# victorramirez952/tomography_3d_reconstructor

Hardware: AMD Instinct MI355X
Metric: Mvoxels/s (SDF+MC) on 1024^3 ellipsoid stack; achieved HBM GB/s vs peak (higher is better)
Workload: dtype f64

## Files before the change

### include/tomo_hip.h

```cpp
#ifndef TOMO_HIP_H
#define TOMO_HIP_H

#include <stddef.h>
#include <stdint.h>

#ifdef __cplusplus
extern "C" {
#endif

#define TOMO_OK 0
#define TOMO_E_ARG (-1)
#define TOMO_E_LAUNCH (-2)
#define TOMO_E_SIZE (-3)
#define TOMO_E_WORKSPACE (-4)

int tomo_abi_version(void);
const char *tomo_error_string(int code);
int tomo_host_mc_cell(const float *h_v, double iso, int8_t *h_tris, int *h_uses_centre);
double tomo_host_mc_edge_offset(double va, double vb);
void tomo_host_mc_centre_offset(const double *h_v8, double *h_out3);

int tomo_host_checksum(const void *h_data, int64_t nbytes, int nthreads, uint64_t *h_out);
int tomo_host_checksum_impl(const void *h_data, int64_t nbytes, int nthreads, int impl, uint64_t *h_out);
int64_t tomo_host_checksum_chunk_bytes(void);
// ... 64 lines not shown
int64_t tomo_mc_scan_workspace_bytes(int64_t n);
int tomo_mc_scan(const uint32_t *counts, int64_t n, uint32_t *off_a, uint32_t *off_b, uint32_t *nz_ids,
                 unsigned long long *totals, void *workspace, int64_t workspace_bytes, void *stream);
int tomo_mc_list(int Nz, int Ny, int Nx, int xorg, const uint32_t *seg_aoff, const unsigned long long *seg_act,
                 unsigned long long *vox_key, void *stream);
int tomo_mc_eval(const float *field, int Nz, int Ny, int Nx, int64_t pitch, int xorg, double iso,
                 const unsigned long long *vox_key, int64_t na, uint32_t *vox_counts, uint8_t *vox_flags, void *stream);
int tomo_mc_list_capped(int Nz, int Ny, int Nx, int xorg, const uint32_t *seg_aoff, const unsigned long long *seg_act,
                        unsigned long long *vox_key, int64_t cap, void *stream);
int tomo_mc_eval_capped(const float *field, int Nz, int Ny, int Nx, int64_t pitch, int xorg, double iso,
                        const unsigned long long *vox_key, int64_t cap, const unsigned long long *na_dev,
                        uint32_t *vox_counts, uint8_t *vox_flags, void *stream);
int tomo_mc_emit(const float *field, int Nz, int Ny, int Nx, int64_t pitch, int xorg, double iso,
                 const unsigned long long *vox_key, int64_t na, const unsigned long long *seg_act,
                 const uint32_t *seg_aoff, const uint32_t *vox_voff, const uint32_t *vox_foff, const uint8_t *vox_flags,
                 int z_offset, unsigned long long *vkey, float *vpos, int32_t *faces, unsigned long long *totals,
                 void *stream);

int tomo_mc_first_touch(const float *field, int Nz, int Ny, int Nx, int64_t pitch, int xorg, double iso,
                        const unsigned long long *vox_key, int64_t na, const unsigned long long *seg_act,
                        const uint32_t *seg_aoff, const uint32_t *vox_voff, const uint8_t *vox_flags, int mode,
                        uint32_t *created, const uint32_t *base, int32_t *ft_rank, unsigned long long *totals, void *stream);

int tomo_mc3_list(int Nz, int Ny, int Nx, int xorg, const uint32_t *seg_cnt, const unsigned long long *seg_act,
                  uint32_t *seg_blk, uint32_t *seg_aoff, unsigned long long *vox_key, int64_t cap, unsigned long long *tot,
                  void *stream);
int tomo_mc3_eval(const float *field, int Nz, int Ny, int Nx, int64_t pitch, int xorg, double iso,
                  const unsigned long long *vox_key, int64_t cap, const unsigned long long *tot, int z_offset,
                  uint32_t *vox_loc, int32_t *vox_til, uint8_t *vox_flags, uint16_t *vox_used, float *vox_f3, float *vox_c3,
                  uint32_t *blk3, void *stream);
int64_t tomo_mc3_slice_table_words(int Nz, int Ny);
int64_t tomo_mc3_sort_segments(int Nz, int Ny);
int tomo_mc3_scan(int Nz, int Ny, int Nx, int xorg, const uint32_t *seg_aoff, const uint32_t *vox_loc, int64_t cap,
                  uint32_t *blk3, uint32_t *slice_tab, unsigned long long *tot, int64_t cap_v, int64_t cap_f, void *stream);
int tomo_mc3_vertices(int Nz, int Ny, int Nx, int xorg, const unsigned long long *vox_key, int64_t cap,
                      const unsigned long long *tot, const uint32_t *vox_loc, const uint8_t *vox_flags, const float *vox_f3,
                      const float *vox_c3, const uint32_t *blk3, const uint32_t *slice_tab, int z_offset, int shift,
                      const double *cum, int64_t ncum, const double *adj, int64_t nadj, float mm_y, float mm_x, float *vrec,
                      uint32_t *keys, uint32_t *idx, void *stream);
int64_t tomo_mc3_sort_workspace_bytes(int64_t cap_v, int64_t nseg);
int tomo_mc3_sort_rank_top(const float *vrec, uint32_t *keys, uint32_t *idx, int64_t cap_v, int Nz, int Ny, const uint32_t *slice_tab,
                           unsigned long long *tot, float *uniq, int32_t *table, void *workspace, int64_t workspace_bytes,
                           float z_top, void *stream);
int tomo_mc3_sort_rank_fused(const float *vrec, const uint32_t *keys, int64_t cap_v, int Nz, int Ny, uint32_t *slice_tab,
                             unsigned long long *tot, float *uniq, int32_t *table, float z_top, void *stream);
int tomo_mc3_faces(int Nz, int Ny, int Nx, int xorg, const unsigned long long *vox_key, int64_t cap, unsigned long long *tot,
// ... 55 lines not shown
```

### tomography_3d_reconstructor_amd/_lib.py

```python
import ctypes
import os
import subprocess

_HERE = os.path.dirname(os.path.abspath(__file__))
SO_PATH = os.environ.get("TOMO_LIB") or os.path.join(_HERE, "libtomo_hip.so")
CSRC = os.path.join(_HERE, "csrc")

_c_i = ctypes.c_int
_c_i64 = ctypes.c_int64
_c_p = ctypes.c_void_p
_c_d = ctypes.c_double
_c_f = ctypes.c_float

SIGNATURES = {
    "tomo_abi_version": (_c_i, []),
    "tomo_error_string": (ctypes.c_char_p, [_c_i]),
    "tomo_host_mc_cell": (_c_i, [_c_p, _c_d, _c_p, _c_p]),
    "tomo_host_mc_edge_offset": (_c_d, [_c_d, _c_d]),
    "tomo_host_mc_centre_offset": (None, [_c_p, _c_p]),
    "tomo_host_checksum": (_c_i, [_c_p, _c_i64, _c_i, _c_p]),
    "tomo_host_checksum_impl": (_c_i, [_c_p, _c_i64, _c_i, _c_i, _c_p]),
    "tomo_host_checksum_chunk_bytes": (_c_i64, []),
    "tomo_host_checksum_part": (_c_i, [_c_p, _c_i64, _c_i64, _c_i, _c_i, _c_p]),
    "tomo_host_checksum_fold": (_c_i, [_c_p, _c_i64, _c_i64, _c_p]),
# ... 33 lines not shown
    "tomo_morph_fused": (_c_i, [_c_p, _c_p, _c_i, _c_i, _c_i, ctypes.c_uint32, _c_i, _c_p]),
    "tomo_smooth": (_c_i, [_c_p, _c_p, _c_i, _c_i, _c_i, _c_i, _c_i, _c_p]),
    "tomo_extend_bits": (_c_i, [_c_p, _c_p, _c_i, _c_i, _c_i, _c_i, _c_p]),
    "tomo_field_fill": (_c_i, [_c_p, _c_p, _c_i, _c_i, _c_i, _c_i, _c_i, _c_p, _c_p, _c_p]),
    "tomo_field_fill_bits": (_c_i, [_c_p, _c_p, _c_i, _c_i, _c_i, _c_i, _c_p, _c_p, _c_p]),
    "tomo_field_span_bytes": (_c_i64, [_c_i, _c_i, _c_i, _c_i]),
    "tomo_field_fill_bits_sparse": (_c_i, [_c_p, _c_p, _c_i, _c_i, _c_i, _c_i, _c_p, _c_p, _c_p, _c_p]),
    "tomo_sign_rows": (_c_i64, [_c_i]),
    "tomo_field_signs_fused": (_c_i, [_c_i]),
    "tomo_sign_buffer_words": (_c_i64, [_c_i, _c_i, _c_i, _c_i]),
    "tomo_field_signs": (_c_i, [_c_p, _c_i, _c_i, _c_i, _c_i64, _c_i, _c_d, _c_i, _c_i, _c_p, _c_p, _c_p]),
    "tomo_mc_classify": (_c_i, [_c_p, _c_p, _c_i, _c_i, _c_i, _c_i, _c_p, _c_p, _c_p]),
    "tomo_mc_scan_segments": (_c_i, [_c_p, _c_i64, _c_p, _c_p, _c_p, _c_i64, _c_p]),
    "tomo_mc_scan_workspace_bytes": (_c_i64, [_c_i64]),
    "tomo_mc_scan": (_c_i, [_c_p, _c_i64, _c_p, _c_p, _c_p, _c_p, _c_p, _c_i64, _c_p]),
    "tomo_mc_list": (_c_i, [_c_i, _c_i, _c_i, _c_i, _c_p, _c_p, _c_p, _c_p]),
    "tomo_mc_eval": (_c_i, [_c_p, _c_i, _c_i, _c_i, _c_i64, _c_i, _c_d, _c_p, _c_i64, _c_p, _c_p, _c_p]),
    "tomo_mc_list_capped": (_c_i, [_c_i, _c_i, _c_i, _c_i, _c_p, _c_p, _c_p, _c_i64, _c_p]),
    "tomo_mc_eval_capped": (_c_i, [_c_p, _c_i, _c_i, _c_i, _c_i64, _c_i, _c_d, _c_p, _c_i64, _c_p, _c_p, _c_p, _c_p]),
    "tomo_mc_emit": (_c_i, [_c_p, _c_i, _c_i, _c_i, _c_i64, _c_i, _c_d, _c_p, _c_i64, _c_p, _c_p, _c_p, _c_p, _c_p, _c_i, _c_p,
                            _c_p, _c_p, _c_p, _c_p]),
    "tomo_mc_first_touch": (_c_i, [_c_p, _c_i, _c_i, _c_i, _c_i64, _c_i, _c_d, _c_p, _c_i64, _c_p, _c_p, _c_p, _c_p, _c_i, _c_p,
                                   _c_p, _c_p, _c_p, _c_p]),
    "tomo_mc3_list": (_c_i, [_c_i, _c_i, _c_i, _c_i, _c_p, _c_p, _c_p, _c_p, _c_p, _c_i64, _c_p, _c_p]),
    "tomo_mc3_eval": (_c_i, [_c_p, _c_i, _c_i, _c_i, _c_i64, _c_i, _c_d, _c_p, _c_i64, _c_p, _c_i, _c_p, _c_p, _c_p, _c_p, _c_p,
                             _c_p, _c_p, _c_p]),
    "tomo_mc3_slice_table_words": (_c_i64, [_c_i, _c_i]),
    "tomo_mc3_sort_segments": (_c_i64, [_c_i, _c_i]),
    "tomo_mc3_scan": (_c_i, [_c_i, _c_i, _c_i, _c_i, _c_p, _c_p, _c_i64, _c_p, _c_p, _c_p, _c_i64, _c_i64, _c_p]),
    "tomo_mc3_vertices": (_c_i, [_c_i, _c_i, _c_i, _c_i, _c_p, _c_i64, _c_p, _c_p, _c_p, _c_p, _c_p, _c_p, _c_p, _c_i, _c_i,
                                 _c_p, _c_i64, _c_p, _c_i64, _c_f, _c_f, _c_p, _c_p, _c_p, _c_p]),
    "tomo_mc3_sort_workspace_bytes": (_c_i64, [_c_i64, _c_i64]),
    "tomo_mc3_sort_rank_top": (_c_i, [_c_p, _c_p, _c_p, _c_i64, _c_i, _c_i, _c_p, _c_p, _c_p, _c_p, _c_p, _c_i64, _c_f, _c_p]),
    "tomo_mc3_sort_rank_fused": (_c_i, [_c_p, _c_p, _c_i64, _c_i, _c_i, _c_p, _c_p, _c_p, _c_p, _c_f, _c_p]),
    "tomo_mc3_faces": (_c_i, [_c_i, _c_i, _c_i, _c_i, _c_p, _c_i64, _c_p, _c_p, _c_p, _c_p, _c_p, _c_p, _c_p, _c_p, _c_p, _c_i64, _c_p]),
    "tomo_vertex_finalize": (_c_i, [_c_p, _c_i64, _c_i, _c_p, _c_i64, _c_p, _c_i64, _c_f, _c_f, _c_p]),
    "tomo_mesh_unique_workspace_bytes": (_c_i64, [_c_i64]),
    "tomo_mesh_unique": (_c_i, [_c_p, _c_i64, _c_p, _c_p, _c_p, _c_p, _c_i64, _c_p]),
    "tomo_mesh_lookup": (_c_i, [_c_p, _c_i64, _c_p, _c_i64, _c_p, _c_p, _c_p]),
    "tomo_slab_top_rows": (_c_i, [_c_p, _c_p, _c_i64, _c_i64, _c_p, _c_p]),
    "tomo_slab_lookup": (_c_i, [_c_p, _c_p, _c_i64, _c_p, _c_i64, _c_p, _c_p, _c_p]),
    "tomo_slab_summary": (_c_i, [_c_p, _c_i64, _c_p, _c_p, _c_i64, _c_i64, _c_p, _c_p]),
    "tomo_slab_lookup_summary": (_c_i, [_c_p, _c_p, _c_i64, _c_p, _c_i64, _c_p, _c_i64, _c_i64, _c_p, _c_p, _c_p]),
    "tomo_mc3_faces_slab": (_c_i, [_c_i, _c_i, _c_i, _c_i, _c_p, _c_i64, _c_p, _c_p, _c_p, _c_p, _c_p, _c_p, _c_p, _c_p, _c_p, _c_i64,
                                   _c_p, _c_i, _c_i, _c_p, _c_i64, _c_i64, _c_p]),
    "tomo_mesh_volume_area": (_c_i, [_c_p, _c_p, _c_i64, _c_p, _c_p]),
# ... 60 lines not shown
```

### tomography_3d_reconstructor_amd/csrc/mc.hip

```cpp
#include <cstring>
#include <cstdlib>
#include "tomo_common.h"
#include <rocprim/rocprim.hpp>

#define MC_LUT_QUAL __device__ const
#define MC_FN __device__ static inline
#include "mc_cell.h"

#define SEG 256
#define KEY_XBITS 20
static_assert(KEY_XBITS + 2 == TOMO_KEY_ROW_SHIFT, "key layout shared with mesh.hip");

struct McGrid {
    int Nz, Ny, Nx;
    int64_t pitch;
    int xorg;
    int segs_per_row;
    double iso;
};

typedef float float4u __attribute__((ext_vector_type(4), aligned(4)));
typedef float float2u __attribute__((ext_vector_type(2), aligned(4)));
typedef float float3u __attribute__((ext_vector_type(3), aligned(4)));
typedef int int3u __attribute__((ext_vector_type(3), aligned(4)));
// ... 37 lines not shown
    u64 b2 = __ballot((double)v[2] > g.iso), b3 = __ballot((double)v[3] > g.iso);
    if (lane < 4)
        signs[((((int64_t)Z * g.segs_per_row + s) * NyP) + Y) * 4 + lane] = lane == 0 ? b0 : (lane == 1 ? b1 : (lane == 2 ? b2 : b3));
}

struct Rec4 { u64 b[4]; };

__device__ static inline Rec4 load_rec(const u64 *__restrict__ signs, int64_t idx)
{
    const ulonglong2 *q = (const ulonglong2 *)(signs + idx * 4);
    ulonglong2 lo = q[0], hi = q[1];
    Rec4 r; r.b[0] = lo.x; r.b[1] = lo.y; r.b[2] = hi.x; r.b[3] = hi.y;
    return r;
}

__device__ static inline Rec4 rec_of(const u64 *__restrict__ signs, int64_t idx, int gc)
{
    if (gc == 2) return load_rec(signs, idx);
    Rec4 r;
    r.b[0] = r.b[1] = r.b[2] = r.b[3] = gc ? ~0ull : 0ull;
    return r;
}

__global__ __launch_bounds__(256) void mc_classify_bits_kernel(const u64 *__restrict__ signs,
                                                               const unsigned char *__restrict__ gcls, const McGrid g,
                                                               int64_t ntasks, u64 *__restrict__ seg_act,
                                                               u32 *__restrict__ seg_cnt)
{
    const int64_t task = (int64_t)blockIdx.x * blockDim.x + threadIdx.x;
    if (task >= ntasks) return;
    int64_t tz, zq;
    const int Y = divmod_pos(task, g.Ny, &tz);
    const int s = divmod_pos(tz, g.segs_per_row, &zq);
    const int Z = (int)zq;
    const int S = g.segs_per_row;
    const int Yn = Y + 1 < g.Ny ? Y + 1 : g.Ny - 1, Z1 = Z + 1 < g.Nz ? Z + 1 : g.Nz - 1;
    const int Xbase = s * SEG - SEG_SHIFT - g.xorg;
    const int64_t segi = ((int64_t)Z * g.Ny + Y) * S + s;
    if (Xbase >= g.Nx || Xbase + SEG <= 0) { seg_cnt[segi] = 0u; return; }
    const bool has_next = s + 1 < S;
    const int64_t NyP = tomo_sign_rows_dev(g.Ny);
    const int64_t ia = ((int64_t)Z * S + s) * NyP + Y, ib = ((int64_t)Z * S + s) * NyP + Yn;
    const int64_t ic = ((int64_t)Z1 * S + s) * NyP + Y, id = ((int64_t)Z1 * S + s) * NyP + Yn;
    const int64_t G = NyP >> 4;
    const int64_t qa = ((int64_t)Z * G + (Y >> 4)) * S + s, qb = ((int64_t)Z * G + (Yn >> 4)) * S + s;
    const int64_t qc = ((int64_t)Z1 * G + (Y >> 4)) * S + s, qd = ((int64_t)Z1 * G + (Yn >> 4)) * S + s;
    const int ga = gcls[qa], gb = gcls[qb], gc = gcls[qc], gd = gcls[qd];
    const int na = has_next ? gcls[qa + 1] : ga, nb = has_next ? gcls[qb + 1] : gb;
    const int nc = has_next ? gcls[qc + 1] : gc, nd = has_next ? gcls[qd + 1] : gd;
    if (ga != 2 && ga == gb && ga == gc && ga == gd && na == ga && nb == ga && nc == ga && nd == ga) {
        seg_cnt[segi] = 0u;
        return;
    }
    Rec4 R[4] = {rec_of(signs, ia, ga), rec_of(signs, ib, gb), rec_of(signs, ic, gc), rec_of(signs, id, gd)};
    u64 nx0[4];
    nx0[0] = has_next ? (na == 2 ? signs[(ia + NyP) * 4] & 1ull : (u64)na) : 0ull;
    nx0[1] = has_next ? (nb == 2 ? signs[(ib + NyP) * 4] & 1ull : (u64)nb) : 0ull;
    nx0[2] = has_next ? (nc == 2 ? signs[(ic + NyP) * 4] & 1ull : (u64)nc) : 0ull;
    nx0[3] = has_next ? (nd == 2 ? signs[(id + NyP) * 4] & 1ull : (u64)nd) : 0ull;
    u64 act[4];
    u64 any_nonzero = 0;
#pragma unroll
    for (int k = 0; k < 4; k++) {
        int lo = Xbase + k < 0 ? (-(Xbase + k) + 3) / 4 : 0;
        int hi = (g.Nx - 1 - Xbase - k) >= 0 ? (g.Nx - 1 - Xbase - k) / 4 : -1;
        if (hi > 63) hi = 63;
        u64 vmask = 0;
        if (hi >= lo) vmask = (hi - lo == 63) ? ~0ull : (((1ull << (hi - lo + 1)) - 1ull) << lo);
        int dl = g.Nx - 1 - Xbase - k;
        u64 lastm = (dl >= 0 && (dl & 3) == 0 && (dl >> 2) < 64) ? (1ull << (dl >> 2)) : 0ull;
        u64 any = 0, all = ~0ull;
#pragma unroll
        for (int r = 0; r < 4; r++) {
            u64 cur = R[r].b[k];
            u64 nxt = k < 3 ? R[r].b[k + 1] : ((R[r].b[0] >> 1) | (nx0[r] << 63));
            nxt = (nxt & ~lastm) | (cur & lastm);
            any |= cur | nxt;
            all &= cur & nxt;
        }
        act[k] = any & ~all & vmask;
        any_nonzero |= act[k];
    }
    seg_cnt[segi] = any_nonzero ? (u32)(__popcll(act[0]) + __popcll(act[1]) + __popcll(act[2]) + __popcll(act[3])) : 0u;
    if (any_nonzero) {
        ulonglong2 *o = (ulonglong2 *)(seg_act + segi * 4);
        o[0] = make_ulonglong2(act[0], act[1]);
        o[1] = make_ulonglong2(act[2], act[3]);
    }
}

static inline int make_grid(McGrid &g, const float *field, int Nz, int Ny, int Nx, int64_t pitch, int xorg, double iso)
{
    if (!field || Nz < 2 || Ny < 2 || Nx < 2 || pitch < Nx + xorg) return TOMO_E_ARG;
    if (Nx >= (1 << KEY_XBITS)) return TOMO_E_SIZE;
    g.Nz = Nz; g.Ny = Ny; g.Nx = Nx; g.pitch = pitch; g.xorg = xorg; g.iso = iso;
    g.segs_per_row = (int)tomo_mc_segments_per_row(Nx, xorg);
    return TOMO_OK;
}

TOMO_API int tomo_field_signs(const float *field, int Nz, int Ny, int Nx, int64_t pitch, int xorg, double iso,
                              int z_begin, int z_end, unsigned long long *signs, uint8_t *gcls, void *stream)
{
    McGrid g;
    int rc = make_grid(g, field, Nz, Ny, Nx, pitch, xorg, iso);
    if (rc) return rc;
    if (!signs || !gcls || z_begin < 0 || z_end > Nz || z_begin > z_end) return TOMO_E_ARG;
    {
        const int64_t per_slice = (tomo_sign_rows(Ny) >> 4) * g.segs_per_row;
        if (z_end > z_begin && hipMemsetAsync(gcls + z_begin * per_slice, 2, (size_t)((z_end - z_begin) * per_slice),
                                              (hipStream_t)stream) != hipSuccess)
            return TOMO_E_LAUNCH;
// ... 505 lines not shown
                                 uint32_t *created,
                                 const uint32_t *base, int32_t *ft_rank, unsigned long long *totals, void *stream)
{
    McGrid g;
    int rc = make_grid(g, field, Nz, Ny, Nx, pitch, xorg, iso);
    if (rc) return rc;
    if (!vox_key || !seg_act || !seg_aoff || !vox_voff || !vox_flags || !totals || (mode == 0 && !created) ||
        (mode == 1 && (!base || !ft_rank)) || (mode != 0 && mode != 1))
        return TOMO_E_ARG;
    if (na <= 0) return TOMO_OK;
    int64_t blocks = ceil_div64(na, 256);
    if (blocks > 0x7fffffff) return TOMO_E_SIZE;
    hipLaunchKernelGGL(mc_first_touch_kernel, dim3((unsigned)blocks), dim3(256), 0, (hipStream_t)stream, field, g,
                       (const u64 *)vox_key, na, (const u64 *)seg_act, seg_aoff, vox_voff, vox_flags, mode, created, base, ft_rank,
                       (u64 *)totals);
    return tomo_status();
}

#define MC3_BLK 256
#define MC3_LOC_A(l) ((l) & 1023u)
#define MC3_LOC_B(l) (((l) >> 10) & 1023u)
#define MC3_LOC_T(l) ((l) >> 20)

__global__ __launch_bounds__(256) void mc3_segsum_kernel(const u32 *__restrict__ seg_cnt, int64_t nseg, u32 *__restrict__ seg_blk,
                                                         int64_t nblk)
{
    const int lane = threadIdx.x & 63;
    const int64_t b = (int64_t)blockIdx.x * 4 + (threadIdx.x >> 6);
    if (b >= nblk) return;
    const int64_t i0 = b * MC3_BLK + lane * 4;
    u32 s = 0;
    if (i0 + 3 < nseg) {
        const uint4 v = *(const uint4 *)(seg_cnt + i0);
        s = v.x + v.y + v.z + v.w;
    } else {
        for (int k = 0; k < 4; k++) if (i0 + k < nseg) s += seg_cnt[i0 + k];
    }
    s = wave_sum(s);
    if (lane == 0) seg_blk[b] = s;
}

template <int K>
__device__ static inline void scan_small_inplace(u32 *__restrict__ a, int64_t stride, int64_t n, u64 *total_out, u32 *lds )
{
    const int lane = threadIdx.x & 63, w = threadIdx.x >> 6;
    u32 carry[K];
    u64 wide[K];
#pragma unroll
    for (int k = 0; k < K; k++) { carry[k] = 0; wide[k] = 0; }
    for (int64_t base = 0; base < n; base += 1024 * 8) {
        const int64_t i0 = base + (int64_t)threadIdx.x * 8;
        u32 v[K][8], s[K];
#pragma unroll
        for (int k = 0; k < K; k++) {
            u32 *p = a + k * stride + i0;
            if (i0 + 7 < n && ((uintptr_t)p & 15) == 0) {
                const uint4 lo = *(const uint4 *)p, hi = *(const uint4 *)(p + 4);
                v[k][0] = lo.x; v[k][1] = lo.y; v[k][2] = lo.z; v[k][3] = lo.w; v[k][4] = hi.x; v[k][5] = hi.y; v[k][6] = hi.z; v[k][7] = hi.w;
            } else {
#pragma unroll
                for (int j = 0; j < 8; j++) v[k][j] = i0 + j < n ? p[j] : 0u;
            }
            s[k] = 0;
#pragma unroll
            for (int j = 0; j < 8; j++) s[k] += v[k][j];
        }
        u32 inc[K];
#pragma unroll
        for (int k = 0; k < K; k++) {
            inc[k] = wave_inclusive_scan(s[k]);
            if (lane == 63) lds[k * 16 + w] = inc[k];
        }
        __syncthreads();
        if (w == 0) {
#pragma unroll
            for (int k = 0; k < K; k++) {
                const u32 t = lane < 16 ? lds[k * 16 + lane] : 0u;
                const u32 ti = wave_inclusive_scan(t);
// ... 4 lines not shown
        __syncthreads();
#pragma unroll
        for (int k = 0; k < K; k++) {
            u32 ex = carry[k] + lds[k * 16 + w] + inc[k] - s[k];
            u32 *p = a + k * stride + i0;
            if (i0 + 7 < n && ((uintptr_t)p & 15) == 0) {
                uint4 lo, hi;
                lo.x = ex; ex += v[k][0]; lo.y = ex; ex += v[k][1]; lo.z = ex; ex += v[k][2]; lo.w = ex; ex += v[k][3];
                hi.x = ex; ex += v[k][4]; hi.y = ex; ex += v[k][5]; hi.z = ex; ex += v[k][6]; hi.w = ex;
                *(uint4 *)p = lo; *(uint4 *)(p + 4) = hi;
            } else {
#pragma unroll
                for (int j = 0; j < 8; j++) { if (i0 + j < n) p[j] = ex; ex += v[k][j]; }
            }
            carry[k] += lds[K * 16 + k];
            wide[k] += lds[K * 16 + k];
        }
        __syncthreads();
    }
#pragma unroll
    for (int k = 0; k < K; k++) total_out[k] = wide[k];
}

__global__ __launch_bounds__(1024) void mc3_scan_seg_kernel(u32 *__restrict__ seg_blk, int64_t nblk, u64 *__restrict__ tot)
{
    __shared__ u32 lds[17];
    u64 total;
    scan_small_inplace<1>(seg_blk, 0, nblk, &total, lds);
    if (threadIdx.x == 0) {
        tot[0] = total;
        tot[1] = tot[2] = tot[4] = tot[5] = tot[6] = tot[7] = 0ull;
        tot[3] = total > 0xffffffffull ? 1ull : 0ull;
    }
}

__global__ __launch_bounds__(MC3_BLK) void mc3_list_kernel(const McGrid g, const u32 *__restrict__ seg_cnt,
                                                           const u32 *__restrict__ seg_blk, const u64 *__restrict__ seg_act,
                                                           int64_t nseg, u32 *__restrict__ seg_aoff, u64 *__restrict__ vox_key,
                                                           u32 cap, u64 *__restrict__ tot)
{
    __shared__ u32 wsum[4];
    const int lane = threadIdx.x & 63, w = threadIdx.x >> 6;
    const int64_t seg = (int64_t)blockIdx.x * MC3_BLK + threadIdx.x;
    const u32 cnt = seg < nseg ? seg_cnt[seg] : 0u;
    const u32 inc = wave_inclusive_scan(cnt);
    if (lane == 63) wsum[w] = inc;
    __syncthreads();
    u32 o = seg_blk[blockIdx.x] + inc - cnt;
    for (int k = 0; k < w; k++) o += wsum[k];
    if (seg >= nseg) return;
    seg_aoff[seg] = o;
    if (seg == nseg - 1) seg_aoff[nseg] = o + cnt;
    if (cnt == 0) return;
    if ((u64)o + cnt > (u64)cap || tot[0] > (u64)cap) {
        if (o <= cap) atomicOr((unsigned long long *)&tot[3], 1ull);
        return;
    }
    int64_t row;
    const int s = divmod_pos(seg, g.segs_per_row, &row);
    const ulonglong2 *q = (const ulonglong2 *)(seg_act + seg * 4);
    const ulonglong2 lo = q[0], hi = q[1];
    const u64 b0 = lo.x, b1 = lo.y, b2 = hi.x, b3 = hi.y;
    const int Xs = s * SEG - SEG_SHIFT - g.xorg;
    u64 any = b0 | b1 | b2 | b3;
    while (any) {
        const int L = __ffsll((long long)any) - 1;
        any &= any - 1;
        const int X0 = Xs + 4 * L;
        if ((b0 >> L) & 1ull) vox_key[o++] = make_key(row, X0, 0);
        if ((b1 >> L) & 1ull) vox_key[o++] = make_key(row, X0 + 1, 0);
        if ((b2 >> L) & 1ull) vox_key[o++] = make_key(row, X0 + 2, 0);
        if ((b3 >> L) & 1ull) vox_key[o++] = make_key(row, X0 + 3, 0);
    }
}

TOMO_API int tomo_mc3_list(int Nz, int Ny, int Nx, int xorg, const uint32_t *seg_cnt, const unsigned long long *seg_act,
                           uint32_t *seg_blk, uint32_t *seg_aoff, unsigned long long *vox_key, int64_t cap,
                           unsigned long long *tot, void *stream)
{
    if (Nz < 2 || Ny < 2 || Nx < 2 || !seg_cnt || !seg_act || !seg_blk || !seg_aoff || !vox_key || !tot) return TOMO_E_ARG;
    if (cap <= 0 || cap >= 0x1fffffffll) return TOMO_E_SIZE;
    if (Nx >= (1 << KEY_XBITS)) return TOMO_E_SIZE;
    McGrid g; g.Nz = Nz; g.Ny = Ny; g.Nx = Nx; g.pitch = 0; g.xorg = xorg; g.iso = 0.0;
    g.segs_per_row = (int)tomo_mc_segments_per_row(Nx, xorg);
    const int64_t nseg = (int64_t)Nz * Ny * g.segs_per_row, nblk = ceil_div64(nseg, MC3_BLK);
    if (nblk > 0x7fffffff) return TOMO_E_SIZE;
    hipStream_t s = (hipStream_t)stream;
    hipLaunchKernelGGL(mc3_segsum_kernel, dim3((unsigned)ceil_div64(nblk, 4)), dim3(256), 0, s, seg_cnt, nseg, seg_blk, nblk);
    hipLaunchKernelGGL(mc3_scan_seg_kernel, dim3(1), dim3(1024), 0, s, seg_blk, nblk, (u64 *)tot);
    hipLaunchKernelGGL(mc3_list_kernel, dim3((unsigned)nblk), dim3(MC3_BLK), 0, s, g, seg_cnt, (const u32 *)seg_blk,
                       (const u64 *)seg_act, nseg, seg_aoff, (u64 *)vox_key, (u32)cap, (u64 *)tot);
    return tomo_status();
}

__global__ __launch_bounds__(MC3_BLK) void mc3_eval_kernel(const float *__restrict__ field, const McGrid g,
                                                           const u64 *__restrict__ vox_key, int64_t cap,
                                                           const u64 *__restrict__ tot, int z_offset,
                                                           u32 *__restrict__ vox_loc, int32_t *__restrict__ vox_til,
                                                           uint8_t *__restrict__ vox_flags, uint16_t *__restrict__ vox_used,
                                                           float *__restrict__ vox_f3, float *__restrict__ vox_c3,
                                                           u32 *__restrict__ blk3, int64_t nblk)
{
    __shared__ u32 wsum[4];
    const int lane = threadIdx.x & 63, w = threadIdx.x >> 6;
    const int64_t i = (int64_t)blockIdx.x * MC3_BLK + threadIdx.x;
    const u64 na = tot[0];
    const bool live = i < cap && (u64)i < na && na <= (u64)cap;
    u32 packed = 0;
    if (live) {
        Cell c;
        load_cell(field, g, vox_key[i], c);
        int ntri = 0;
        int32_t til = 0;
        u32 used = 0;
// ... 26 lines not shown
        packed = (u32)__popc(c.flags & 3) | ((u32)__popc(c.flags & 12) << 10) | ((u32)ntri << 20);
    }
    const u32 inc = wave_inclusive_scan(packed);
    if (lane == 63) wsum[w] = inc;
    __syncthreads();
    u32 ex = inc - packed;
    for (int k = 0; k < w; k++) ex += wsum[k];
    if (i < cap) vox_loc[i] = ex;
    if (threadIdx.x == MC3_BLK - 1) {
        const u32 sum = ex + packed;
        blk3[blockIdx.x] = MC3_LOC_A(sum);
        blk3[nblk + blockIdx.x] = MC3_LOC_B(sum);
        blk3[2 * nblk + blockIdx.x] = MC3_LOC_T(sum);
    }
}

__global__ __launch_bounds__(1024) void mc3_scan_kernel(const McGrid g, const u32 *__restrict__ seg_aoff,
                                                        const u32 *__restrict__ vox_loc, int64_t cap, u32 *__restrict__ blk3,
                                                        int64_t nblk, u32 *__restrict__ slice_tab, u64 *__restrict__ tot,
                                                        int64_t cap_v, int64_t cap_f)
{
    __shared__ u32 lds[3 * 16 + 3];
    u64 totals[3];
    scan_small_inplace<3>(blk3, nblk, nblk, totals, lds);
    const u64 na = tot[0];
    const u64 totA64 = totals[0], totB64 = totals[1], totT64 = totals[2];
    const u32 totA = (u32)totA64, totB = (u32)totB64;
    const int Nz = g.Nz;
    u32 *sliceA = slice_tab, *sliceB = slice_tab + (Nz + 1);
    const int64_t segs_per_slice = (int64_t)g.Ny * g.segs_per_row;
    const bool fits = na <= (u64)cap;
    for (int Z = threadIdx.x; Z <= Nz; Z += 1024) {
        u32 a = totA, b = totB;
        if (Z < Nz && fits) {
            const u64 s = seg_aoff[(int64_t)Z * segs_per_slice];
            if (s < na) {
                const u32 l = vox_loc[s];
                a = blk3[s >> 8] + MC3_LOC_A(l);
                b = blk3[nblk + (s >> 8)] + MC3_LOC_B(l);
            }
        }
        sliceA[Z] = a;
        sliceB[Z] = b;
    }
    u64 ov = 0;
    if (totA64 + totB64 > (u64)cap_v) ov |= 2ull;
    if (totT64 > (u64)cap_f) ov |= 4ull;
// ... 316 lines not shown
```

### tomography_3d_reconstructor_amd/pipeline.py

```python
import math
import os
import threading
from dataclasses import dataclass

import numpy as np
import torch

from . import _lib


COUNTERS = dict.fromkeys(("na_hint_hit", "na_hint_miss", "mc3_hint_hit", "mc3_hint_miss", "mc3_sort_fused", "mc3_sort_library",
                          "mc3_exact", "mc3_general_unique", "mc3_degenerate"), 0)
NA_HINTS = os.environ.get("TOMO_NA_HINTS", "1") not in ("", "0")
_NA_HINT = {}
LIST_LIMIT = 2 ** 31
MESH_LIMIT = 2 ** 31
PACK_CLOSE_FUSED = os.environ.get("TOMO_PACK_CLOSE", "1") not in ("", "0")
FIELD_FROM_BITS = True
FIELD_SPARSE = os.environ.get("TOMO_FIELD_SPARSE", "0") not in ("", "0")


def _stream():
    return torch.cuda.current_stream().cuda_stream

# ... 461 lines not shown
class Mc3Surface:

    def __init__(self, f, slice_depths, mm_per_pixel_y, mm_per_pixel_x, add_padding=True, z_offset=0, z_top=None, tot=None):
        self.field, self.z_offset = f, int(z_offset)
        self.z_top = float("nan") if z_top is None else float(z_top)
        self.hint_key = (f.Nz, f.Ny, f.Nx, self.z_offset)
        self._depth = _depth_args(slice_depths, add_padding, f.data.device)
        self._mm = (float(np.float32(mm_per_pixel_y)), float(np.float32(mm_per_pixel_x)))
        self.tot = torch.empty(8, dtype=torch.int64, device=f.data.device) if tot is None else tot
        self.uniq = self.table = self.faces_final = None
        self.nv = self.nf = self.na = 0
        self.deferred = False
        self._pending = None

    def classify(self):
        L, f, dev = _lib.lib(), self.field, self.field.data.device
        if f.signs is None or f.signs_level != 0.5:
            if f.sparse:
                raise _lib.TomoError("a sparse field holds floats only near the 0.5 surface")
            field_signs(f, 0.5)
        nseg = f.Nz * f.Ny * L.tomo_mc_segments_per_row(f.Nx, f.xorg)
        self.seg_act = torch.empty(nseg * 4, dtype=torch.int64, device=dev)
        self.seg_cnt = torch.empty(nseg, dtype=torch.int32, device=dev)
        _lib.check(L.tomo_mc_classify(_p(f.signs), _p(f.gcls), f.Nz, f.Ny, f.Nx, f.xorg, _p(self.seg_act), _p(self.seg_cnt), _stream()),
                   "tomo_mc_classify")
        self.seg_blk = torch.empty((nseg + 255) // 256, dtype=torch.int32, device=dev)
        self.seg_aoff = torch.empty(nseg + 1, dtype=torch.int32, device=dev)

    def build_list(self, cap):
        f, self.cap = self.field, cap
        self.vox_key = torch.empty(cap, dtype=torch.int64, device=f.data.device)
        _lib.check(_lib.lib().tomo_mc3_list(f.Nz, f.Ny, f.Nx, f.xorg, _p(self.seg_cnt), _p(self.seg_act), _p(self.seg_blk), _p(self.seg_aoff),
                                            _p(self.vox_key), cap, _p(self.tot), _stream()), "tomo_mc3_list")

    def eval_scan(self, cap_v, cap_f):
        L, f, cap, st, dev = _lib.lib(), self.field, self.cap, _stream(), self.field.data.device
        self.vox_loc = torch.empty(cap, dtype=torch.int32, device=dev)
        self.vox_til = torch.empty(cap, dtype=torch.int32, device=dev)
        self.vox_flags = torch.empty(cap, dtype=torch.uint8, device=dev)
        self.vox_used = torch.empty(cap, dtype=torch.int16, device=dev)
        self.vox_f3 = torch.empty(3 * cap, dtype=torch.float32, device=dev)
        self.vox_c3 = torch.empty(3 * cap, dtype=torch.float32, device=dev)
        self.blk3 = torch.empty(3 * ((cap + 255) // 256), dtype=torch.int32, device=dev)
        self.slice_tab = torch.empty(L.tomo_mc3_slice_table_words(f.Nz, f.Ny), dtype=torch.int32, device=dev)
        _lib.check(L.tomo_mc3_eval(_p(f.data), f.Nz, f.Ny, f.Nx, f.pitch, f.xorg, 0.5, _p(self.vox_key), cap, _p(self.tot), self.z_offset,
                                   _p(self.vox_loc), _p(self.vox_til), _p(self.vox_flags), _p(self.vox_used), _p(self.vox_f3),
                                   _p(self.vox_c3), _p(self.blk3), st), "tomo_mc3_eval")
        _lib.check(L.tomo_mc3_scan(f.Nz, f.Ny, f.Nx, f.xorg, _p(self.seg_aoff), _p(self.vox_loc), cap, _p(self.blk3), _p(self.slice_tab),
                                   _p(self.tot), cap_v, cap_f, st), "tomo_mc3_scan")
# ... 443 lines not shown
```

Baseline: 690,200.

## Classify only live 16-row strips and fuse segment counting into hierarchical strip sums

Adds a compaction pass that uses the coarse group classes to list only the 16-row strip groups that may contain the surface. Only those strips run the per-segment classification, and the same pass accumulates per-strip and per-superstrip counts with atomics, which removes the separate segment-sum kernel. The list kernel now scans one strip per wave using these hierarchical offsets instead of scanning per 256-segment block. The cost is a memset of the whole seg_cnt array, an extra launch, and atomic contention; dead strips still get their offsets written.

```diff
diff --git a/include/tomo_hip.h b/include/tomo_hip.h
--- a/include/tomo_hip.h
+++ b/include/tomo_hip.h
@@ -110,6 +110,10 @@
                         const uint32_t *seg_aoff, const uint32_t *vox_voff, const uint8_t *vox_flags, int mode,
                         uint32_t *created, const uint32_t *base, int32_t *ft_rank, unsigned long long *totals, void *stream);
 
+int64_t tomo_mc3_strip_words(int Nz, int Ny);
+int64_t tomo_mc3_work_words(int Nz, int Ny, int Nx, int xorg);
+int tomo_mc3_classify(const unsigned long long *signs, const uint8_t *gcls, int Nz, int Ny, int Nx, int xorg,
+                      unsigned long long *seg_act, uint32_t *seg_cnt, uint32_t *seg_blk, uint32_t *work, void *stream);
 int tomo_mc3_list(int Nz, int Ny, int Nx, int xorg, const uint32_t *seg_cnt, const unsigned long long *seg_act,
                   uint32_t *seg_blk, uint32_t *seg_aoff, unsigned long long *vox_key, int64_t cap, unsigned long long *tot,
                   void *stream);
diff --git a/tomography_3d_reconstructor_amd/_lib.py b/tomography_3d_reconstructor_amd/_lib.py
--- a/tomography_3d_reconstructor_amd/_lib.py
+++ b/tomography_3d_reconstructor_amd/_lib.py
@@ -79,6 +79,9 @@
                             _c_p, _c_p, _c_p, _c_p]),
     "tomo_mc_first_touch": (_c_i, [_c_p, _c_i, _c_i, _c_i, _c_i64, _c_i, _c_d, _c_p, _c_i64, _c_p, _c_p, _c_p, _c_p, _c_i, _c_p,
                                    _c_p, _c_p, _c_p, _c_p]),
+    "tomo_mc3_strip_words": (_c_i64, [_c_i, _c_i]),
+    "tomo_mc3_work_words": (_c_i64, [_c_i, _c_i, _c_i, _c_i]),
+    "tomo_mc3_classify": (_c_i, [_c_p, _c_p, _c_i, _c_i, _c_i, _c_i, _c_p, _c_p, _c_p, _c_p, _c_p]),
     "tomo_mc3_list": (_c_i, [_c_i, _c_i, _c_i, _c_i, _c_p, _c_p, _c_p, _c_p, _c_p, _c_i64, _c_p, _c_p]),
     "tomo_mc3_eval": (_c_i, [_c_p, _c_i, _c_i, _c_i, _c_i64, _c_i, _c_d, _c_p, _c_i64, _c_p, _c_i, _c_p, _c_p, _c_p, _c_p, _c_p,
                              _c_p, _c_p, _c_p]),
diff --git a/tomography_3d_reconstructor_amd/csrc/mc.hip b/tomography_3d_reconstructor_amd/csrc/mc.hip
--- a/tomography_3d_reconstructor_amd/csrc/mc.hip
+++ b/tomography_3d_reconstructor_amd/csrc/mc.hip
@@ -83,22 +83,14 @@
     return r;
 }
 
-__global__ __launch_bounds__(256) void mc_classify_bits_kernel(const u64 *__restrict__ signs,
-                                                               const unsigned char *__restrict__ gcls, const McGrid g,
-                                                               int64_t ntasks, u64 *__restrict__ seg_act,
-                                                               u32 *__restrict__ seg_cnt)
-{
-    const int64_t task = (int64_t)blockIdx.x * blockDim.x + threadIdx.x;
-    if (task >= ntasks) return;
-    int64_t tz, zq;
-    const int Y = divmod_pos(task, g.Ny, &tz);
-    const int s = divmod_pos(tz, g.segs_per_row, &zq);
-    const int Z = (int)zq;
+__device__ static inline u32 classify_segment(const u64 *__restrict__ signs, const unsigned char *__restrict__ gcls,
+                                              const McGrid &g, int Z, int Y, int s, u64 *__restrict__ seg_act)
+{
     const int S = g.segs_per_row;
     const int Yn = Y + 1 < g.Ny ? Y + 1 : g.Ny - 1, Z1 = Z + 1 < g.Nz ? Z + 1 : g.Nz - 1;
     const int Xbase = s * SEG - SEG_SHIFT - g.xorg;
     const int64_t segi = ((int64_t)Z * g.Ny + Y) * S + s;
-    if (Xbase >= g.Nx || Xbase + SEG <= 0) { seg_cnt[segi] = 0u; return; }
+    if (Xbase >= g.Nx || Xbase + SEG <= 0) return 0u;
     const bool has_next = s + 1 < S;
     const int64_t NyP = tomo_sign_rows_dev(g.Ny);
     const int64_t ia = ((int64_t)Z * S + s) * NyP + Y, ib = ((int64_t)Z * S + s) * NyP + Yn;
@@ -109,10 +101,8 @@
     const int ga = gcls[qa], gb = gcls[qb], gc = gcls[qc], gd = gcls[qd];
     const int na = has_next ? gcls[qa + 1] : ga, nb = has_next ? gcls[qb + 1] : gb;
     const int nc = has_next ? gcls[qc + 1] : gc, nd = has_next ? gcls[qd + 1] : gd;
-    if (ga != 2 && ga == gb && ga == gc && ga == gd && na == ga && nb == ga && nc == ga && nd == ga) {
-        seg_cnt[segi] = 0u;
-        return;
-    }
+    if (ga != 2 && ga == gb && ga == gc && ga == gd && na == ga && nb == ga && nc == ga && nd == ga)
+        return 0u;
     Rec4 R[4] = {rec_of(signs, ia, ga), rec_of(signs, ib, gb), rec_of(signs, ic, gc), rec_of(signs, id, gd)};
     u64 nx0[4];
     nx0[0] = has_next ? (na == 2 ? signs[(ia + NyP) * 4] & 1ull : (u64)na) : 0ull;
@@ -142,12 +132,25 @@
         act[k] = any & ~all & vmask;
         any_nonzero |= act[k];
     }
-    seg_cnt[segi] = any_nonzero ? (u32)(__popcll(act[0]) + __popcll(act[1]) + __popcll(act[2]) + __popcll(act[3])) : 0u;
-    if (any_nonzero) {
-        ulonglong2 *o = (ulonglong2 *)(seg_act + segi * 4);
-        o[0] = make_ulonglong2(act[0], act[1]);
-        o[1] = make_ulonglong2(act[2], act[3]);
-    }
+    if (!any_nonzero) return 0u;
+    ulonglong2 *o = (ulonglong2 *)(seg_act + segi * 4);
+    o[0] = make_ulonglong2(act[0], act[1]);
+    o[1] = make_ulonglong2(act[2], act[3]);
+    return (u32)(__popcll(act[0]) + __popcll(act[1]) + __popcll(act[2]) + __popcll(act[3]));
+}
+
+__global__ __launch_bounds__(256) void mc_classify_bits_kernel(const u64 *__restrict__ signs,
+                                                               const unsigned char *__restrict__ gcls, const McGrid g,
+                                                               int64_t ntasks, u64 *__restrict__ seg_act,
+                                                               u32 *__restrict__ seg_cnt)
+{
+    const int64_t task = (int64_t)blockIdx.x * blockDim.x + threadIdx.x;
+    if (task >= ntasks) return;
+    int64_t tz, zq;
+    const int Y = divmod_pos(task, g.Ny, &tz);
+    const int s = divmod_pos(tz, g.segs_per_row, &zq);
+    const int Z = (int)zq;
+    seg_cnt[((int64_t)Z * g.Ny + Y) * g.segs_per_row + s] = classify_segment(signs, gcls, g, Z, Y, s, seg_act);
 }
 
 static inline int make_grid(McGrid &g, const float *field, int Nz, int Ny, int Nx, int64_t pitch, int xorg, double iso)
@@ -699,26 +702,118 @@
 #define MC3_LOC_B(l) (((l) >> 10) & 1023u)
 #define MC3_LOC_T(l) ((l) >> 20)
 
-__global__ __launch_bounds__(256) void mc3_segsum_kernel(const u32 *__restrict__ seg_cnt, int64_t nseg, u32 *__restrict__ seg_blk,
-                                                         int64_t nblk)
+struct Mc3Strips { int64_t nstrip, nstripP, nsup, nsupP; };
+
+static inline Mc3Strips mc3_strips(int Nz, int Ny)
+{
+    Mc3Strips t;
+    t.nstrip = (int64_t)Nz * (tomo_sign_rows(Ny) >> 4);
+    t.nstripP = ceil_div64(t.nstrip, 64) * 64;
+    t.nsup = t.nstripP / 64;
+    t.nsupP = ceil_div64(t.nsup, 4) * 4;
+    return t;
+}
+
+TOMO_API int64_t tomo_mc3_strip_words(int Nz, int Ny)
+{
+    if (Nz < 1 || Ny < 1) return 0;
+    const Mc3Strips t = mc3_strips(Nz, Ny);
+    return t.nstripP + 2 * t.nsupP;
+}
+
+TOMO_API int64_t tomo_mc3_work_words(int Nz, int Ny, int Nx, int xorg)
+{
+    if (Nz < 1 || Ny < 1 || Nx < 1) return 0;
+    return (int64_t)Nz * (tomo_sign_rows(Ny) >> 4) * tomo_mc_segments_per_row(Nx, xorg) + 1;
+}
+
+__global__ __launch_bounds__(256) void mc3_live_kernel(const unsigned char *__restrict__ gcls, const McGrid g, int64_t ngroups,
+                                                       u32 *__restrict__ seg_blk, int64_t nzero, u32 *__restrict__ work)
 {
     const int lane = threadIdx.x & 63;
-    const int64_t b = (int64_t)blockIdx.x * 4 + (threadIdx.x >> 6);
-    if (b >= nblk) return;
-    const int64_t i0 = b * MC3_BLK + lane * 4;
-    u32 s = 0;
-    if (i0 + 3 < nseg) {
-        const uint4 v = *(const uint4 *)(seg_cnt + i0);
-        s = v.x + v.y + v.z + v.w;
-    } else {
-        for (int k = 0; k < 4; k++) if (i0 + k < nseg) s += seg_cnt[i0 + k];
-    }
-    s = wave_sum(s);
-    if (lane == 0) seg_blk[b] = s;
+    const int64_t q = (int64_t)blockIdx.x * 256 + threadIdx.x;
+    for (int64_t i = q; i < nzero; i += (int64_t)gridDim.x * 256) seg_blk[i] = 0u;
+    bool live = false;
+    if (q < ngroups) {
+        const int S = g.segs_per_row, G = (int)(tomo_sign_rows_dev(g.Ny) >> 4);
+        int64_t zy, zq;
+        const int s = divmod_pos(q, S, &zy);
+        const int yg = divmod_pos(zy, G, &zq);
+        const int Z = (int)zq;
+        const int Xbase = s * SEG - SEG_SHIFT - g.xorg;
+        if (Xbase < g.Nx && Xbase + SEG > 0) {
+            const int c = gcls[q];
+            live = c == 2;
+            if (!live) {
+                const int Yl = yg * 16 + 15 < g.Ny ? yg * 16 + 15 : g.Ny - 1;
+                const int Yn = Yl + 1 < g.Ny ? Yl + 1 : g.Ny - 1, Z1 = Z + 1 < g.Nz ? Z + 1 : g.Nz - 1;
+                const int64_t qb = ((int64_t)Z * G + (Yn >> 4)) * S + s;
+                const int64_t qc = ((int64_t)Z1 * G + yg) * S + s, qd = ((int64_t)Z1 * G + (Yn >> 4)) * S + s;
+                live = gcls[qb] != c || gcls[qc] != c || gcls[qd] != c;
+                if (!live && s + 1 < S) live = gcls[q + 1] != c || gcls[qb + 1] != c || gcls[qc + 1] != c || gcls[qd + 1] != c;
+            }
+        }
+    }
+    const u64 m = __ballot(live);
+    if (m == 0) return;
+    const int leader = __ffsll((long long)m) - 1;
+    u32 base = 0;
+    if (lane == leader) base = atomicAdd(&work[0], (u32)__popcll(m));
+    base = __shfl(base, leader, 64);
+    if (live) work[1 + base + (u32)__popcll(m & ((1ull << lane) - 1ull))] = (u32)q;
+}
+
+__global__ __launch_bounds__(256) void mc3_classify_live_kernel(const u64 *__restrict__ signs, const unsigned char *__restrict__ gcls,
+                                                                const McGrid g, const u32 *__restrict__ work,
+                                                                u64 *__restrict__ seg_act, u32 *__restrict__ seg_cnt,
+                                                                u32 *__restrict__ strip_cnt, u32 *__restrict__ sup_cnt)
+{
+    const u32 nlive = work[0];
+    if (blockIdx.x * 16u >= nlive) return;
+    const u32 slot = blockIdx.x * 16u + (threadIdx.x >> 4);
+    u32 cnt = 0;
+    int64_t strip = 0;
+    if (slot < nlive) {
+        const int S = g.segs_per_row, G = (int)(tomo_sign_rows_dev(g.Ny) >> 4);
+        const int s = divmod_pos((int64_t)work[1 + slot], S, &strip);
+        int64_t zq;
+        const int yg = divmod_pos(strip, G, &zq);
+        const int Z = (int)zq, Y = yg * 16 + (int)(threadIdx.x & 15);
+        if (Y < g.Ny) {
+            cnt = classify_segment(signs, gcls, g, Z, Y, s, seg_act);
+            if (cnt) seg_cnt[((int64_t)Z * g.Ny + Y) * S + s] = cnt;
+        }
+    }
+#pragma unroll
+    for (int d = 8; d > 0; d >>= 1) cnt += __shfl_xor(cnt, d, 64);
+    if ((threadIdx.x & 15) == 0 && cnt) {
+        atomicAdd(&strip_cnt[strip], cnt);
+        atomicAdd(&sup_cnt[strip >> 6], cnt);
+    }
+}
+
+TOMO_API int tomo_mc3_classify(const unsigned long long *signs, const uint8_t *gcls, int Nz, int Ny, int Nx, int xorg,
+                               unsigned long long *seg_act, uint32_t *seg_cnt, uint32_t *seg_blk, uint32_t *work, void *stream)
+{
+    if (!signs || !gcls || !seg_act || !seg_cnt || !seg_blk || !work || Nz < 2 || Ny < 2 || Nx < 2) return TOMO_E_ARG;
+    if (Nx >= (1 << KEY_XBITS)) return TOMO_E_SIZE;
+    McGrid g; g.Nz = Nz; g.Ny = Ny; g.Nx = Nx; g.pitch = 0; g.xorg = xorg; g.iso = 0.0;
+    g.segs_per_row = (int)tomo_mc_segments_per_row(Nx, xorg);
+    const Mc3Strips t = mc3_strips(Nz, Ny);
+    const int64_t nseg = (int64_t)Nz * Ny * g.segs_per_row, ngroups = t.nstrip * g.segs_per_row;
+    if (ngroups > 0x7fffffff) return TOMO_E_SIZE;
+    hipStream_t s = (hipStream_t)stream;
+    if (hipMemsetAsync(work, 0, sizeof(u32), s) != hipSuccess) return TOMO_E_LAUNCH;
+    if (hipMemsetAsync(seg_cnt, 0, (size_t)nseg * sizeof(u32), s) != hipSuccess) return TOMO_E_LAUNCH;
+    hipLaunchKernelGGL(mc3_live_kernel, dim3((unsigned)ceil_div64(ngroups, 256)), dim3(256), 0, s, gcls, g, ngroups, seg_blk,
+                       t.nstripP + t.nsupP, work);
+    hipLaunchKernelGGL(mc3_classify_live_kernel, dim3((unsigned)ceil_div64(ngroups, 16)), dim3(256), 0, s, (const u64 *)signs, gcls,
+                       g, (const u32 *)work, (u64 *)seg_act, seg_cnt, seg_blk, seg_blk + t.nstripP);
+    return tomo_status();
 }
 
 template <int K>
-__device__ static inline void scan_small_inplace(u32 *__restrict__ a, int64_t stride, int64_t n, u64 *total_out, u32 *lds )
+__device__ static inline void scan_small(const u32 *src, u32 *a, int64_t stride, int64_t n, u64 *total_out, u32 *lds )
 {
     const int lane = threadIdx.x & 63, w = threadIdx.x >> 6;
     u32 carry[K];
@@ -730,7 +825,7 @@
         u32 v[K][8], s[K];
 #pragma unroll
         for (int k = 0; k < K; k++) {
-            u32 *p = a + k * stride + i0;
+            const u32 *p = src + k * stride + i0;
             if (i0 + 7 < n && ((uintptr_t)p & 15) == 0) {
                 const uint4 lo = *(const uint4 *)p, hi = *(const uint4 *)(p + 4);
                 v[k][0] = lo.x; v[k][1] = lo.y; v[k][2] = lo.z; v[k][3] = lo.w; v[k][4] = hi.x; v[k][5] = hi.y; v[k][6] = hi.z; v[k][7] = hi.w;
@@ -781,11 +876,12 @@
     for (int k = 0; k < K; k++) total_out[k] = wide[k];
 }
 
-__global__ __launch_bounds__(1024) void mc3_scan_seg_kernel(u32 *__restrict__ seg_blk, int64_t nblk, u64 *__restrict__ tot)
+__global__ __launch_bounds__(1024) void mc3_scan_seg_kernel(const u32 *__restrict__ sup_cnt, u32 *__restrict__ sup_off, int64_t nsup,
+                                                            u64 *__restrict__ tot)
 {
     __shared__ u32 lds[17];
     u64 total;
-    scan_small_inplace<1>(seg_blk, 0, nblk, &total, lds);
+    scan_small<1>(sup_cnt, sup_off, 0, nsup, &total, lds);
     if (threadIdx.x == 0) {
         tot[0] = total;
         tot[1] = tot[2] = tot[4] = tot[5] = tot[6] = tot[7] = 0ull;
@@ -794,42 +890,59 @@
 }
 
 __global__ __launch_bounds__(MC3_BLK) void mc3_list_kernel(const McGrid g, const u32 *__restrict__ seg_cnt,
-                                                           const u32 *__restrict__ seg_blk, const u64 *__restrict__ seg_act,
-                                                           int64_t nseg, u32 *__restrict__ seg_aoff, u64 *__restrict__ vox_key,
-                                                           u32 cap, u64 *__restrict__ tot)
-{
-    __shared__ u32 wsum[4];
-    const int lane = threadIdx.x & 63, w = threadIdx.x >> 6;
-    const int64_t seg = (int64_t)blockIdx.x * MC3_BLK + threadIdx.x;
-    const u32 cnt = seg < nseg ? seg_cnt[seg] : 0u;
-    const u32 inc = wave_inclusive_scan(cnt);
-    if (lane == 63) wsum[w] = inc;
-    __syncthreads();
-    u32 o = seg_blk[blockIdx.x] + inc - cnt;
-    for (int k = 0; k < w; k++) o += wsum[k];
-    if (seg >= nseg) return;
-    seg_aoff[seg] = o;
-    if (seg == nseg - 1) seg_aoff[nseg] = o + cnt;
-    if (cnt == 0) return;
-    if ((u64)o + cnt > (u64)cap || tot[0] > (u64)cap) {
-        if (o <= cap) atomicOr((unsigned long long *)&tot[3], 1ull);
+                                                           const u32 *__restrict__ strip_cnt, const u32 *__restrict__ sup_off,
+                                                           const u64 *__restrict__ seg_act, int64_t nstrip,
+                                                           u32 *__restrict__ seg_aoff, u64 *__restrict__ vox_key, u32 cap,
+                                                           u64 *__restrict__ tot)
+{
+    const int lane = threadIdx.x & 63;
+    const int64_t strip = (int64_t)blockIdx.x * 4 + (threadIdx.x >> 6);
+    if (strip >= nstrip) return;
+    const int S = g.segs_per_row, G = (int)(tomo_sign_rows_dev(g.Ny) >> 4);
+    int64_t Z;
+    const int yg = divmod_pos(strip, G, &Z);
+    const int rows = g.Ny - yg * 16 < 16 ? g.Ny - yg * 16 : 16;
+    const int64_t row0 = Z * g.Ny + yg * 16, seg0 = row0 * S;
+    const int n = rows * S;
+    const u32 mine = strip_cnt[(strip & ~(int64_t)63) + lane];
+    const u32 inc = wave_inclusive_scan(mine);
+    const u32 base = sup_off[strip >> 6] + __shfl(inc - mine, (int)(strip & 63), 64);
+    const u32 total = __shfl(mine, (int)(strip & 63), 64);
+    if (strip == nstrip - 1 && lane == 0) seg_aoff[seg0 + n] = base + total;
+    if (total == 0) {
+        for (int i = lane; i < n; i += 64) seg_aoff[seg0 + i] = base;
         return;
     }
-    int64_t row;
-    const int s = divmod_pos(seg, g.segs_per_row, &row);
-    const ulonglong2 *q = (const ulonglong2 *)(seg_act + seg * 4);
-    const ulonglong2 lo = q[0], hi = q[1];
-    const u64 b0 = lo.x, b1 = lo.y, b2 = hi.x, b3 = hi.y;
-    const int Xs = s * SEG - SEG_SHIFT - g.xorg;
-    u64 any = b0 | b1 | b2 | b3;
-    while (any) {
-        const int L = __ffsll((long long)any) - 1;
-        any &= any - 1;
-        const int X0 = Xs + 4 * L;
-        if ((b0 >> L) & 1ull) vox_key[o++] = make_key(row, X0, 0);
-        if ((b1 >> L) & 1ull) vox_key[o++] = make_key(row, X0 + 1, 0);
-        if ((b2 >> L) & 1ull) vox_key[o++] = make_key(row, X0 + 2, 0);
-        if ((b3 >> L) & 1ull) vox_key[o++] = make_key(row, X0 + 3, 0);
+    const bool too_long = tot[0] > (u64)cap;
+    u32 carry = base;
+    for (int i0 = 0; i0 < n; i0 += 64) {
+        const int i = i0 + lane;
+        const u32 cnt = i < n ? seg_cnt[seg0 + i] : 0u;
+        const u32 ic = wave_inclusive_scan(cnt);
+        u32 o = carry + ic - cnt;
+        carry += __shfl(ic, 63, 64);
+        if (i < n) seg_aoff[seg0 + i] = o;
+        if (cnt == 0) {
+        } else if ((u64)o + cnt > (u64)cap || too_long) {
+            if (o <= cap) atomicOr((unsigned long long *)&tot[3], 1ull);
+        } else {
+            const int r = i / S, s = i - r * S;
+            const int64_t row = row0 + r;
+            const ulonglong2 *q = (const ulonglong2 *)(seg_act + (seg0 + i) * 4);
+            const ulonglong2 lo = q[0], hi = q[1];
+            const u64 b0 = lo.x, b1 = lo.y, b2 = hi.x, b3 = hi.y;
+            const int Xs = s * SEG - SEG_SHIFT - g.xorg;
+            u64 any = b0 | b1 | b2 | b3;
+            while (any) {
+                const int L = __ffsll((long long)any) - 1;
+                any &= any - 1;
+                const int X0 = Xs + 4 * L;
+                if ((b0 >> L) & 1ull) vox_key[o++] = make_key(row, X0, 0);
+                if ((b1 >> L) & 1ull) vox_key[o++] = make_key(row, X0 + 1, 0);
+                if ((b2 >> L) & 1ull) vox_key[o++] = make_key(row, X0 + 2, 0);
+                if ((b3 >> L) & 1ull) vox_key[o++] = make_key(row, X0 + 3, 0);
+            }
+        }
     }
 }
 
@@ -842,13 +955,13 @@
     if (Nx >= (1 << KEY_XBITS)) return TOMO_E_SIZE;
     McGrid g; g.Nz = Nz; g.Ny = Ny; g.Nx = Nx; g.pitch = 0; g.xorg = xorg; g.iso = 0.0;
     g.segs_per_row = (int)tomo_mc_segments_per_row(Nx, xorg);
-    const int64_t nseg = (int64_t)Nz * Ny * g.segs_per_row, nblk = ceil_div64(nseg, MC3_BLK);
-    if (nblk > 0x7fffffff) return TOMO_E_SIZE;
+    const Mc3Strips t = mc3_strips(Nz, Ny);
+    if (ceil_div64(t.nstrip, 4) > 0x7fffffff) return TOMO_E_SIZE;
     hipStream_t s = (hipStream_t)stream;
-    hipLaunchKernelGGL(mc3_segsum_kernel, dim3((unsigned)ceil_div64(nblk, 4)), dim3(256), 0, s, seg_cnt, nseg, seg_blk, nblk);
-    hipLaunchKernelGGL(mc3_scan_seg_kernel, dim3(1), dim3(1024), 0, s, seg_blk, nblk, (u64 *)tot);
-    hipLaunchKernelGGL(mc3_list_kernel, dim3((unsigned)nblk), dim3(MC3_BLK), 0, s, g, seg_cnt, (const u32 *)seg_blk,
-                       (const u64 *)seg_act, nseg, seg_aoff, (u64 *)vox_key, (u32)cap, (u64 *)tot);
+    uint32_t *sup_cnt = seg_blk + t.nstripP, *sup_off = sup_cnt + t.nsupP;
+    hipLaunchKernelGGL(mc3_scan_seg_kernel, dim3(1), dim3(1024), 0, s, (const u32 *)sup_cnt, sup_off, t.nsup, (u64 *)tot);
+    hipLaunchKernelGGL(mc3_list_kernel, dim3((unsigned)ceil_div64(t.nstrip, 4)), dim3(MC3_BLK), 0, s, g, seg_cnt, (const u32 *)seg_blk,
+                       (const u32 *)sup_off, (const u64 *)seg_act, t.nstrip, seg_aoff, (u64 *)vox_key, (u32)cap, (u64 *)tot);
     return tomo_status();
 }
 
@@ -921,7 +1034,7 @@
 {
     __shared__ u32 lds[3 * 16 + 3];
     u64 totals[3];
-    scan_small_inplace<3>(blk3, nblk, nblk, totals, lds);
+    scan_small<3>(blk3, blk3, nblk, nblk, totals, lds);
     const u64 na = tot[0];
     const u64 totA64 = totals[0], totB64 = totals[1], totT64 = totals[2];
     const u32 totA = (u32)totA64, totB = (u32)totB64;
diff --git a/tomography_3d_reconstructor_amd/pipeline.py b/tomography_3d_reconstructor_amd/pipeline.py
--- a/tomography_3d_reconstructor_amd/pipeline.py
+++ b/tomography_3d_reconstructor_amd/pipeline.py
@@ -507,9 +507,10 @@
         nseg = f.Nz * f.Ny * L.tomo_mc_segments_per_row(f.Nx, f.xorg)
         self.seg_act = torch.empty(nseg * 4, dtype=torch.int64, device=dev)
         self.seg_cnt = torch.empty(nseg, dtype=torch.int32, device=dev)
-        _lib.check(L.tomo_mc_classify(_p(f.signs), _p(f.gcls), f.Nz, f.Ny, f.Nx, f.xorg, _p(self.seg_act), _p(self.seg_cnt), _stream()),
-                   "tomo_mc_classify")
-        self.seg_blk = torch.empty((nseg + 255) // 256, dtype=torch.int32, device=dev)
+        self.seg_blk = torch.empty(L.tomo_mc3_strip_words(f.Nz, f.Ny), dtype=torch.int32, device=dev)
+        work = torch.empty(L.tomo_mc3_work_words(f.Nz, f.Ny, f.Nx, f.xorg), dtype=torch.int32, device=dev)
+        _lib.check(L.tomo_mc3_classify(_p(f.signs), _p(f.gcls), f.Nz, f.Ny, f.Nx, f.xorg, _p(self.seg_act), _p(self.seg_cnt),
+                                       _p(self.seg_blk), _p(work), _stream()), "tomo_mc3_classify")
         self.seg_aoff = torch.empty(nseg + 1, dtype=torch.int32, device=dev)
 
     def build_list(self, cap):
```

Measured after the change: 664,200. -3.8%, worse.
